# ViacheslavDanilov/oct_segmentation

Hardware: AMD Instinct MI355X
Metric: OCT frames/sec (704x704, bf16) fwd+bwd (higher is better)
Workload: dtype bf16; 1 GPU; unetplusplus/resnet101 1-class 704x704, batch 16/GPU, fwd+Dice+bwd+allreduce+Adam; global_batch=16, parallelism=dp1

## Files before the change

### oct_segmentation_amd/csrc/gemm1x1.hip

```cpp
#include "common.h"
#include "conv_common.h"
#include "kernels.h"

#include <cstdlib>
#include <type_traits>

namespace octseg {

constexpr int G1_BM = 128;
constexpr int G1_D = 3;
constexpr int G1_MAXWG = 512;

struct G1Args {
  const char* x; long long xstride;
  const float* scale; const float* shift; int relu;
  const char* w;
  char* y; long long ystride; int accum;
  int M, K, N, n_tiles, m_tiles;
  float* slab; int slab_row0;
  const float* bias; int relu_out;
};

template <typename T, int NT, bool AFF, bool BRES>
__global__ __launch_bounds__(256, BRES ? 1 : 2) void gemm1x1_kernel(const G1Args a) {
  constexpr int D = BRES ? 6 : G1_D;
  constexpr int NSET = D + 1;
  constexpr int NSLOT = BRES ? 4 : 2;
  constexpr int BN = NT * 32;
  constexpr int SLAB = BN * 128;
  constexpr int NPB = SLAB / 4096;
  constexpr int OPITCH = BN * 2 + 16;
  constexpr int PPR = BN / 8;
  constexpr int RPI = 64 / PPR;
  extern __shared__ __attribute__((aligned(16))) char smem[];
  char* ldsB = smem;
  char* strip0 = smem + NSLOT * SLAB;
  float* lds_ss = (float*)(strip0 + 4 * 32 * OPITCH);

  const int tid = threadIdx.x, lane = tid & 63, wave = tid >> 6;
  const int r = lane & 31, h = lane >> 5;
  const int G = gridDim.x;
  const int wid = blockIdx.x;
  const int l = (G & 7) == 0 ? (wid & 7) * (G >> 3) + (wid >> 3) : wid;
  const int nt_idx = l % a.n_tiles, wg_m = l / a.n_tiles, Gm = G / a.n_tiles;
  const int nloc = (a.m_tiles - wg_m + Gm - 1) / Gm;
  const int S = a.K >> 6;
  const int total = nloc * S;
  const int n0 = nt_idx * BN;

  if constexpr (AFF) {
    for (int k = tid; k < a.K; k += 256) { lds_ss[k] = a.scale[k]; lds_ss[a.K + k] = a.shift[k]; }
  }

  int pf_s = 0, pf_mt = wg_m;
  auto row_ptr = [&](int mt) -> const char* {
    const int row = min(mt * G1_BM + wave * 32 + r, a.M - 1);
    return a.x + (long long)row * a.xstride + 64 * h;
  };
  const char* pf_ptr = row_ptr(pf_mt);
  uint4 A[NSET][4];
  auto load_A = [&](uint4 (&dst)[4]) __attribute__((always_inline)) {
#pragma unroll
    for (int j = 0; j < 4; ++j) dst[j] = *(const uint4*)(pf_ptr + 16 * j);
    pf_ptr += 128;
    if (++pf_s == S) {
      pf_s = 0;
      if (pf_mt + Gm < a.m_tiles) pf_mt += Gm;
      pf_ptr = row_ptr(pf_mt);
    }
  };
  int bs = 0;
  const char* wbase = a.w + (long long)nt_idx * SLAB + tid * 16;
  const long long wstep = (long long)a.n_tiles * SLAB;
  uint4 B0 = make_uint4(0, 0, 0, 0), B1 = B0, B2 = B0, B3 = B0;
#define G1_LOAD_B()                                                        \
  do {                                                                     \
    const char* p_ = wbase + bs * wstep;                                   \
    B0 = *(const uint4*)(p_);                                              \
    if constexpr (NPB > 1) B1 = *(const uint4*)(p_ + 4096);                \
    if constexpr (NPB > 2) { B2 = *(const uint4*)(p_ + 8192); B3 = *(const uint4*)(p_ + 12288); } \
    if (++bs == S) bs = 0;                                                 \
  } while (0)
#define G1_STORE_B(slot_)                                                  \
  do {                                                                     \
    char* q_ = ldsB + (slot_) * SLAB + tid * 16;                           \
    *(uint4*)(q_) = B0;                                                    \
    if constexpr (NPB > 1) *(uint4*)(q_ + 4096) = B1;                      \
    if constexpr (NPB > 2) { *(uint4*)(q_ + 8192) = B2; *(uint4*)(q_ + 12288) = B3; } \
  } while (0)

  f32x16_t acc[NT];
#pragma unroll
  for (int nt = 0; nt < NT; ++nt)
#pragma unroll
    for (int v = 0; v < 16; ++v) acc[nt][v] = 0.f;
  float s1[NT], s2[NT];
#pragma unroll
  for (int nt = 0; nt < NT; ++nt) { s1[nt] = 0.f; s2[nt] = 0.f; }

  float obias[NT];
#pragma unroll
  for (int nt = 0; nt < NT; ++nt) obias[nt] = (a.bias != nullptr && n0 + nt * 32 + r < a.N) ? a.bias[n0 + nt * 32 + r] : 0.f;
  const float ofloor = a.relu_out ? 0.f : NO_FLOOR;
  const int bswz = (r >> 1) & 7;
  const int bbase = r * 128;
  const unsigned floor16 = a.relu ? 0u : 0x80008000u;

  if constexpr (BRES) {
    for (int q = 0; q < S; ++q) { G1_LOAD_B(); G1_STORE_B(q); }
  } else {
    G1_LOAD_B();
    G1_STORE_B(0);
    G1_LOAD_B();
  }
#pragma unroll
  for (int d = 0; d < D; ++d) load_A(A[d]);
  __syncthreads();

  int s = 0, mt = wg_m;
  char* strip = strip0 + wave * 32 * OPITCH;

  auto epilogue = [&]() __attribute__((always_inline)) {
    const int m0 = mt * G1_BM + wave * 32;
    if (a.bias != nullptr) {
#pragma unroll
      for (int nt = 0; nt < NT; ++nt)
#pragma unroll
        for (int v = 0; v < 16; ++v) acc[nt][v] = clamp_lo(acc[nt][v] + obias[nt], ofloor);
    }
    if (a.slab != nullptr) {
#pragma unroll
      for (int nt = 0; nt < NT; ++nt)
#pragma unroll
        for (int v = 0; v < 16; ++v) { const float y = acc[nt][v]; s1[nt] += y; s2[nt] += y * y; }
    }
#pragma unroll
    for (int nt = 0; nt < NT; ++nt)
#pragma unroll
      for (int v = 0; v < 16; ++v) {
        const int row = (v & 3) + 8 * (v >> 2) + 4 * h;
        Tr<T>::store(strip + row * OPITCH, nt * 32 + r, acc[nt][v]);
        acc[nt][v] = 0.f;
      }
    __builtin_amdgcn_fence(__ATOMIC_RELEASE, "wavefront");
    asm volatile("s_waitcnt lgkmcnt(0)" ::: "memory");
    const int piece = lane % PPR, rsub = lane / PPR;
    const int n = n0 + piece * 8;
    const bool nok = n < a.N;
    char* gp0 = a.y + (long long)(m0 + rsub) * a.ystride + n * 2;
    const long long gstep = (long long)RPI * a.ystride;
    if (a.accum) {
      uint4 old[32 / RPI];
#pragma unroll
      for (int i = 0; i < 32 / RPI; ++i) {
        const bool ok = nok && m0 + rsub + i * RPI < a.M;
        old[i] = *(const uint4*)(ok ? gp0 + i * gstep : (char*)a.y);
      }
#pragma unroll
      for (int i = 0; i < 32 / RPI; ++i) {
        const int row = rsub + i * RPI;
        if (nok && m0 + row < a.M) {
          const uint4 val = *(const uint4*)(strip + row * OPITCH + piece * 16);
          float x0[8], x1[8];
          Tr<T>::unpack8(val, x0); Tr<T>::unpack8(old[i], x1);
#pragma unroll
          for (int e = 0; e < 8; ++e) x0[e] += x1[e];
          *(uint4*)(gp0 + i * gstep) = Tr<T>::pack8(x0);
        }
      }
    } else {
#pragma unroll
      for (int i = 0; i < 32 / RPI; ++i) {
        const int row = rsub + i * RPI;
        if (nok && m0 + row < a.M) *(uint4*)(gp0 + i * gstep) = *(const uint4*)(strip + row * OPITCH + piece * 16);
      }
    }
    asm volatile("s_waitcnt lgkmcnt(0)" ::: "memory");
  };

  auto step = [&](auto set_c, int g) __attribute__((always_inline)) {
    constexpr int SET = decltype(set_c)::value;
    const int slot = BRES ? s : (g & 1);
    if constexpr (!BRES) {
      G1_STORE_B(slot ^ 1);
      G1_LOAD_B();
    }
    load_A(A[(SET + D) % NSET]);
    const bool tail = (mt * G1_BM + G1_BM > a.M);
    const bool valid = mt * G1_BM + wave * 32 + r < a.M;
    const char* bsl = ldsB + slot * SLAB + bbase;
    uint4 bf[2][NT];
#pragma unroll
    for (int nt = 0; nt < NT; ++nt) bf[0][nt] = *(const uint4*)(bsl + nt * 4096 + (((4 * h + 0) ^ bswz) * 16));
#pragma unroll
    for (int j = 0; j < 4; ++j) {
      if (j + 1 < 4) {
#pragma unroll
        for (int nt = 0; nt < NT; ++nt) bf[(j + 1) & 1][nt] = *(const uint4*)(bsl + nt * 4096 + (((4 * h + j + 1) ^ bswz) * 16));
      }
      uint4 af = A[SET][j];
      if constexpr (AFF) {
        const int k0 = s * 64 + 32 * h + 8 * j;
        float sc[8], sh[8];
        const float4 c0 = *(const float4*)(lds_ss + k0), c1 = *(const float4*)(lds_ss + k0 + 4);
        const float4 d0 = *(const float4*)(lds_ss + a.K + k0), d1 = *(const float4*)(lds_ss + a.K + k0 + 4);
        sc[0] = c0.x; sc[1] = c0.y; sc[2] = c0.z; sc[3] = c0.w; sc[4] = c1.x; sc[5] = c1.y; sc[6] = c1.z; sc[7] = c1.w;
        sh[0] = d0.x; sh[1] = d0.y; sh[2] = d0.z; sh[3] = d0.w; sh[4] = d1.x; sh[5] = d1.y; sh[6] = d1.z; sh[7] = d1.w;
        af = Tr<T>::affine_floor(af, sc, sh, floor16);
      }
      if (tail && !valid) af = make_uint4(0, 0, 0, 0);
      __builtin_amdgcn_sched_barrier(0);
#pragma unroll
      for (int nt = 0; nt < NT; ++nt) Tr<T>::mma(af, bf[j & 1][nt], acc[nt]);
      __builtin_amdgcn_sched_barrier(0);
    }
    if (++s == S) {
      epilogue();
      s = 0;
      mt += Gm;
    }
    if constexpr (!BRES) __syncthreads();
  };

  for (int g = 0; g < total; g += NSET) {
    step(std::integral_constant<int, 0>{}, g);
    if (g + 1 < total) step(std::integral_constant<int, 1>{}, g + 1);
    if (g + 2 < total) step(std::integral_constant<int, 2>{}, g + 2);
    if (g + 3 < total) step(std::integral_constant<int, 3>{}, g + 3);
    if constexpr (NSET > 4) {
      if (g + 4 < total) step(std::integral_constant<int, 4 % NSET>{}, g + 4);
      if (g + 5 < total) step(std::integral_constant<int, 5 % NSET>{}, g + 5);
      if (g + 6 < total) step(std::integral_constant<int, 6 % NSET>{}, g + 6);
    }
  }
  if constexpr (BRES) __syncthreads();

#undef G1_LOAD_B
#undef G1_STORE_B
  if (a.slab != nullptr) {
    float* red = (float*)strip0;
#pragma unroll
    for (int nt = 0; nt < NT; ++nt) {
      s1[nt] += __shfl_xor(s1[nt], 32);
      s2[nt] += __shfl_xor(s2[nt], 32);
      if (h == 0) { red[(wave * BN + nt * 32 + r) * 2] = s1[nt]; red[(wave * BN + nt * 32 + r) * 2 + 1] = s2[nt]; }
    }
    __syncthreads();
    if (tid < BN && n0 + tid < a.N) {
      float t1 = 0.f, t2 = 0.f;
#pragma unroll
      for (int w = 0; w < 4; ++w) { t1 += red[(w * BN + tid) * 2]; t2 += red[(w * BN + tid) * 2 + 1]; }
      float* o = a.slab + ((size_t)(a.slab_row0 + wg_m) * a.N + n0 + tid) * 2;
      o[0] = t1; o[1] = t2;
    }
  }
}

namespace {

struct G1Geom { int NT, n_tiles, m_tiles, G, rows, bres; size_t lds; };

static G1Geom g1_geom(const ConvArgs& a) {
  G1Geom g;
  g.NT = a.Cout > 64 ? 4 : (a.Cout > 32 ? 2 : 1);
  const int BN = g.NT * 32;
  g.n_tiles = (a.Cout + BN - 1) / BN;
  const long long M = (long long)a.N * a.OH * a.OW;
  g.m_tiles = (int)((M + G1_BM - 1) / G1_BM);
  static const bool use_bres = getenv("OCTSEG_G1_BRES") != nullptr;
  g.bres = (use_bres && g.NT == 4 && a.Cin <= 256 && a.Cin >= 128 && g.n_tiles >= 4) ? 1 : 0;
  int gm = (g.bres ? G1_MAXWG / 2 : G1_MAXWG) / g.n_tiles;
  if (gm < 1) gm = 1;
  if (gm > g.m_tiles) gm = g.m_tiles;
  g.rows = gm;
  g.G = gm * g.n_tiles;
  const bool aff = a.src[0].scale != nullptr;
  g.lds = (size_t)(g.bres ? 4 : 2) * BN * 128 + (size_t)4 * 32 * (BN * 2 + 16) + (aff ? (size_t)a.Cin * 8 : 0);
  return g;
}

}

bool gemm1x1_eligible(const ConvArgs& a, int dtype) {
  static const bool off = getenv("OCTSEG_NO_GEMM1X1") != nullptr;
  if (off || dtype == DT_F32) return false;
  if (a.ntaps != 1 || a.istride != 1 || a.ostride != 1 || a.out_mode == OUT_HEAD_NCHW) return false;
  if (a.tap_dy[0] != 0 || a.tap_dx[0] != 0 || a.nsrc != 1 || a.ndst != 1) return false;
  if (a.bias != nullptr && a.stat_slab != nullptr) return false;
  const SrcDesc& s = a.src[0];
  const DstDesc& d = a.dst[0];
  if (s.up || s.C != a.Cin || s.c0 != 0 || s.H != a.IH || s.W != a.IW || a.IH != a.OH || a.IW != a.OW) return false;
  if (d.pool || d.c0 != 0 || d.H != a.OH || d.W != a.OW || d.cn != a.Cout) return false;
  if (a.Cin % 64 != 0 || a.Cin > 4096 || a.Cout % 8 != 0 || a.Cout < 8) return false;
  if ((long long)a.N * a.OH * a.OW < 1) return false;
  return true;
}

int gemm1x1_rows(const ConvArgs& a) { return g1_geom(a).rows; }

template <typename T, int NT, bool AFF, bool BRES>
static hipError_t g1_launch_k(const G1Args& ga, const G1Geom& g, hipStream_t st) {
  static bool set = false;
  if (!set) {
    hipError_t e = hipFuncSetAttribute((const void*)gemm1x1_kernel<T, NT, AFF, BRES>, hipFuncAttributeMaxDynamicSharedMemorySize, 160 * 1024);
    if (e != hipSuccess) return e;
    set = true;
  }
  hipLaunchKernelGGL((gemm1x1_kernel<T, NT, AFF, BRES>), dim3(g.G), dim3(256), g.lds, st, ga);
  return hipGetLastError();
}
template <typename T, int NT>
static hipError_t g1_launch(const G1Args& ga, const G1Geom& g, bool aff, hipStream_t st) {
  if constexpr (NT == 4) {
    if (g.bres) return aff ? g1_launch_k<T, NT, true, true>(ga, g, st) : g1_launch_k<T, NT, false, true>(ga, g, st);
  }
  return aff ? g1_launch_k<T, NT, true, false>(ga, g, st) : g1_launch_k<T, NT, false, false>(ga, g, st);
}

hipError_t launch_gemm1x1(int dtype, const ConvArgs& a, hipStream_t st) {
  const G1Geom g = g1_geom(a);
  G1Args ga;
  const SrcDesc& s = a.src[0];
  const DstDesc& d = a.dst[0];
  ga.x = (const char*)s.ptr; ga.xstride = (long long)s.C * 2;
  ga.scale = s.scale; ga.shift = s.shift; ga.relu = s.relu;
  ga.w = (const char*)a.W;
  ga.y = (char*)d.ptr; ga.ystride = (long long)d.C * 2; ga.accum = (d.accum || a.out_mode == OUT_ACCUM) ? 1 : 0;
  ga.M = (int)((long long)a.N * a.OH * a.OW); ga.K = a.Cin; ga.N = a.Cout; ga.n_tiles = g.n_tiles; ga.m_tiles = g.m_tiles;
  ga.slab = a.stat_slab; ga.slab_row0 = a.slab_row0;
  ga.bias = a.bias; ga.relu_out = a.relu_out;
  const bool aff = s.scale != nullptr;
  if (dtype == DT_F16) {
    switch (g.NT) {
      case 4: return g1_launch<f16_t, 4>(ga, g, aff, st);
      case 2: return g1_launch<f16_t, 2>(ga, g, aff, st);
      default: return g1_launch<f16_t, 1>(ga, g, aff, st);
    }
  }
  switch (g.NT) {
    case 4: return g1_launch<bf16_t, 4>(ga, g, aff, st);
    case 2: return g1_launch<bf16_t, 2>(ga, g, aff, st);
    default: return g1_launch<bf16_t, 1>(ga, g, aff, st);
  }
}

}
```

Measured before the change: 254.9 frames/s.

## Add three-slot LDS ring with direct global-to-LDS weight loads in 1x1 GEMM

Adds a RING variant of the 1x1 GEMM kernel that streams weight tiles straight into a three-slot LDS ring using global_load_lds_dwordx4, skipping the register round trip. Activations are loaded with inline-asm global loads and waited on with explicit vmcnt counters, so each step needs only a single s_barrier. The epilogue strip is narrowed to write half the N tile at a time, which keeps LDS within the 80KB cap. It is enabled by default whenever it fits that cap. The hand-written waitcnt and m0 handling are fragile and depend on the exact order the compiler emits instructions.

```diff
diff --git a/oct_segmentation_amd/csrc/gemm1x1.hip b/oct_segmentation_amd/csrc/gemm1x1.hip
--- a/oct_segmentation_amd/csrc/gemm1x1.hip
+++ b/oct_segmentation_amd/csrc/gemm1x1.hip
@@ -21,23 +21,30 @@
   const float* bias; int relu_out;
 };
 
-template <typename T, int NT, bool AFF, bool BRES>
+constexpr int g1_ring_ew(int NT) { return NT == 4 ? 2 : NT; }
+constexpr int G1_RING_SLOTS = 3;
+constexpr size_t G1_RING_LDS_MAX = 80 * 1024;
+
+template <typename T, int NT, bool AFF, bool BRES, bool RING>
 __global__ __launch_bounds__(256, BRES ? 1 : 2) void gemm1x1_kernel(const G1Args a) {
+  static_assert(!(BRES && RING), "one weight pipeline per instantiation");
+  typedef __attribute__((ext_vector_type(4))) unsigned u32x4_t;
   constexpr int D = BRES ? 6 : G1_D;
   constexpr int NSET = D + 1;
-  constexpr int NSLOT = BRES ? 4 : 2;
+  constexpr int NSLOT = BRES ? 4 : (RING ? G1_RING_SLOTS : 2);
   constexpr int BN = NT * 32;
   constexpr int SLAB = BN * 128;
   constexpr int NPB = SLAB / 4096;
-  constexpr int OPITCH = BN * 2 + 16;
-  constexpr int PPR = BN / 8;
+  constexpr int EW = RING ? g1_ring_ew(NT) : NT;
+  constexpr int OPITCH = EW * 64 + 16;
+  constexpr int PPR = EW * 4;
   constexpr int RPI = 64 / PPR;
   extern __shared__ __attribute__((aligned(16))) char smem[];
   char* ldsB = smem;
   char* strip0 = smem + NSLOT * SLAB;
   float* lds_ss = (float*)(strip0 + 4 * 32 * OPITCH);
 
-  const int tid = threadIdx.x, lane = tid & 63, wave = tid >> 6;
+  const int tid = threadIdx.x, lane = tid & 63, wave = __builtin_amdgcn_readfirstlane(tid >> 6);
   const int r = lane & 31, h = lane >> 5;
   const int G = gridDim.x;
   const int wid = blockIdx.x;
@@ -69,9 +76,35 @@
       pf_ptr = row_ptr(pf_mt);
     }
   };
+  u32x4_t RA[NSET][4];
+  auto load_RA = [&](u32x4_t (&dst)[4]) __attribute__((always_inline)) {
+    asm volatile("global_load_dwordx4 %0, %1, off" : "=v"(dst[0]) : "v"(pf_ptr));
+    asm volatile("global_load_dwordx4 %0, %1, off offset:16" : "=v"(dst[1]) : "v"(pf_ptr));
+    asm volatile("global_load_dwordx4 %0, %1, off offset:32" : "=v"(dst[2]) : "v"(pf_ptr));
+    asm volatile("global_load_dwordx4 %0, %1, off offset:48" : "=v"(dst[3]) : "v"(pf_ptr));
+    pf_ptr += 128;
+    if (++pf_s == S) {
+      pf_s = 0;
+      if (pf_mt + Gm < a.m_tiles) pf_mt += Gm;
+      pf_ptr = row_ptr(pf_mt);
+    }
+  };
   int bs = 0;
   const char* wbase = a.w + (long long)nt_idx * SLAB + tid * 16;
   const long long wstep = (long long)a.n_tiles * SLAB;
+  const unsigned ldsB_addr = (unsigned)(size_t)(__attribute__((address_space(3))) char*)ldsB;
+  auto dma_B = [&](int slot) __attribute__((always_inline)) {
+    const char* p_ = wbase + bs * wstep;
+#pragma unroll
+    for (int i = 0; i < NPB; ++i) {
+      const char* g_ = p_ + i * 4096;
+      const unsigned dst = __builtin_amdgcn_readfirstlane(ldsB_addr + (unsigned)slot * SLAB + (unsigned)i * 4096u + (unsigned)wave * 1024u);
+      unsigned keep;
+      asm volatile("s_mov_b32 %0, m0\n\ts_mov_b32 m0, %2\n\ts_nop 0\n\tglobal_load_lds_dwordx4 %1, off\n\ts_mov_b32 m0, %0"
+                   : "=&s"(keep) : "v"(g_), "s"(dst) : "memory");
+    }
+    if (++bs == S) bs = 0;
+  };
   uint4 B0 = make_uint4(0, 0, 0, 0), B1 = B0, B2 = B0, B3 = B0;
 #define G1_LOAD_B()                                                        \
   do {                                                                     \
@@ -106,16 +139,29 @@
   const int bbase = r * 128;
   const unsigned floor16 = a.relu ? 0u : 0x80008000u;
 
-  if constexpr (BRES) {
-    for (int q = 0; q < S; ++q) { G1_LOAD_B(); G1_STORE_B(q); }
+  if constexpr (RING) {
+#pragma unroll
+    for (int nt = 0; nt < NT; ++nt) asm volatile("" : "+v"(obias[nt]));
+    asm volatile("s_waitcnt vmcnt(0)" ::: "memory");
+    load_RA(RA[0]); dma_B(0);
+    load_RA(RA[1]); dma_B(1);
+    load_RA(RA[2]);
+    asm volatile("s_waitcnt vmcnt(%4)" : "+v"(RA[0][0]), "+v"(RA[0][1]), "+v"(RA[0][2]), "+v"(RA[0][3]) : "n"(8 + NPB) : "memory");
+    asm volatile("s_waitcnt lgkmcnt(0)" ::: "memory");
+    __builtin_amdgcn_s_barrier();
+    asm volatile("" ::: "memory");
   } else {
-    G1_LOAD_B();
-    G1_STORE_B(0);
-    G1_LOAD_B();
-  }
-#pragma unroll
-  for (int d = 0; d < D; ++d) load_A(A[d]);
-  __syncthreads();
+    if constexpr (BRES) {
+      for (int q = 0; q < S; ++q) { G1_LOAD_B(); G1_STORE_B(q); }
+    } else {
+      G1_LOAD_B();
+      G1_STORE_B(0);
+      G1_LOAD_B();
+    }
+#pragma unroll
+    for (int d = 0; d < D; ++d) load_A(A[d]);
+    __syncthreads();
+  }
 
   int s = 0, mt = wg_m;
   char* strip = strip0 + wave * 32 * OPITCH;
@@ -135,17 +181,19 @@
         for (int v = 0; v < 16; ++v) { const float y = acc[nt][v]; s1[nt] += y; s2[nt] += y * y; }
     }
 #pragma unroll
-    for (int nt = 0; nt < NT; ++nt)
+    for (int ep = 0; ep < NT / EW; ++ep) {
+#pragma unroll
+    for (int e = 0; e < EW; ++e)
 #pragma unroll
       for (int v = 0; v < 16; ++v) {
         const int row = (v & 3) + 8 * (v >> 2) + 4 * h;
-        Tr<T>::store(strip + row * OPITCH, nt * 32 + r, acc[nt][v]);
-        acc[nt][v] = 0.f;
+        Tr<T>::store(strip + row * OPITCH, e * 32 + r, acc[ep * EW + e][v]);
+        acc[ep * EW + e][v] = 0.f;
       }
     __builtin_amdgcn_fence(__ATOMIC_RELEASE, "wavefront");
     asm volatile("s_waitcnt lgkmcnt(0)" ::: "memory");
     const int piece = lane % PPR, rsub = lane / PPR;
-    const int n = n0 + piece * 8;
+    const int n = n0 + ep * EW * 32 + piece * 8;
     const bool nok = n < a.N;
     char* gp0 = a.y + (long long)(m0 + rsub) * a.ystride + n * 2;
     const long long gstep = (long long)RPI * a.ystride;
@@ -168,6 +216,8 @@
           *(uint4*)(gp0 + i * gstep) = Tr<T>::pack8(x0);
         }
       }
+#pragma unroll
+      for (int i = 0; i < 32 / RPI; ++i) asm volatile("" :: "v"(old[i].x), "v"(old[i].y), "v"(old[i].z), "v"(old[i].w));
     } else {
 #pragma unroll
       for (int i = 0; i < 32 / RPI; ++i) {
@@ -176,16 +226,10 @@
       }
     }
     asm volatile("s_waitcnt lgkmcnt(0)" ::: "memory");
-  };
-
-  auto step = [&](auto set_c, int g) __attribute__((always_inline)) {
-    constexpr int SET = decltype(set_c)::value;
-    const int slot = BRES ? s : (g & 1);
-    if constexpr (!BRES) {
-      G1_STORE_B(slot ^ 1);
-      G1_LOAD_B();
-    }
-    load_A(A[(SET + D) % NSET]);
+    }
+  };
+
+  auto compute = [&](const uint4 (&a4)[4], int slot) __attribute__((always_inline)) {
     const bool tail = (mt * G1_BM + G1_BM > a.M);
     const bool valid = mt * G1_BM + wave * 32 + r < a.M;
     const char* bsl = ldsB + slot * SLAB + bbase;
@@ -198,7 +242,7 @@
 #pragma unroll
         for (int nt = 0; nt < NT; ++nt) bf[(j + 1) & 1][nt] = *(const uint4*)(bsl + nt * 4096 + (((4 * h + j + 1) ^ bswz) * 16));
       }
-      uint4 af = A[SET][j];
+      uint4 af = a4[j];
       if constexpr (AFF) {
         const int k0 = s * 64 + 32 * h + 8 * j;
         float sc[8], sh[8];
@@ -214,6 +258,17 @@
       for (int nt = 0; nt < NT; ++nt) Tr<T>::mma(af, bf[j & 1][nt], acc[nt]);
       __builtin_amdgcn_sched_barrier(0);
     }
+  };
+
+  auto step = [&](auto set_c, int g) __attribute__((always_inline)) {
+    constexpr int SET = decltype(set_c)::value;
+    const int slot = BRES ? s : (g & 1);
+    if constexpr (!BRES) {
+      G1_STORE_B(slot ^ 1);
+      G1_LOAD_B();
+    }
+    load_A(A[(SET + D) % NSET]);
+    compute(A[SET], slot);
     if (++s == S) {
       epilogue();
       s = 0;
@@ -222,6 +277,42 @@
     if constexpr (!BRES) __syncthreads();
   };
 
+  int rslot = 0, wslot = 2;
+  auto rstep = [&](auto set_c, bool live) __attribute__((always_inline)) {
+    constexpr int SET = decltype(set_c)::value;
+    constexpr int NXT = (SET + 1) % NSET;
+    dma_B(wslot);
+    if (++wslot == NSLOT) wslot = 0;
+    load_RA(RA[(SET + D) % NSET]);
+    uint4 a4[4];
+#pragma unroll
+    for (int j = 0; j < 4; ++j) a4[j] = __builtin_bit_cast(uint4, RA[SET][j]);
+    if (live) compute(a4, rslot);
+    if (++rslot == NSLOT) rslot = 0;
+    asm volatile("s_waitcnt vmcnt(%4)" : "+v"(RA[NXT][0]), "+v"(RA[NXT][1]), "+v"(RA[NXT][2]), "+v"(RA[NXT][3]) : "n"(8 + NPB) : "memory");
+    if (live && ++s == S) {
+      epilogue();
+      s = 0;
+      mt += Gm;
+    }
+    asm volatile("s_waitcnt lgkmcnt(0)" ::: "memory");
+    __builtin_amdgcn_s_barrier();
+    asm volatile("" ::: "memory");
+  };
+
+  if constexpr (RING) {
+    static_assert(NSET == 4, "the unrolled ring walk below");
+    for (int g = 0; g < total; g += NSET) {
+      rstep(std::integral_constant<int, 0>{}, true);
+      rstep(std::integral_constant<int, 1>{}, g + 1 < total);
+      rstep(std::integral_constant<int, 2>{}, g + 2 < total);
+      rstep(std::integral_constant<int, 3>{}, g + 3 < total);
+    }
+    asm volatile("s_waitcnt vmcnt(0)"
+                 : "+v"(RA[0][0]), "+v"(RA[0][1]), "+v"(RA[0][2]), "+v"(RA[0][3]), "+v"(RA[1][0]), "+v"(RA[1][1]), "+v"(RA[1][2]), "+v"(RA[1][3]),
+                   "+v"(RA[2][0]), "+v"(RA[2][1]), "+v"(RA[2][2]), "+v"(RA[2][3]), "+v"(RA[3][0]), "+v"(RA[3][1]), "+v"(RA[3][2]), "+v"(RA[3][3])
+                 :: "memory");
+  } else
   for (int g = 0; g < total; g += NSET) {
     step(std::integral_constant<int, 0>{}, g);
     if (g + 1 < total) step(std::integral_constant<int, 1>{}, g + 1);
@@ -258,7 +349,11 @@
 
 namespace {
 
-struct G1Geom { int NT, n_tiles, m_tiles, G, rows, bres; size_t lds; };
+struct G1Geom { int NT, n_tiles, m_tiles, G, rows, bres, ring; size_t lds; };
+
+static size_t g1_lds_bytes(int NT, int slots, int ew, bool aff, int K) {
+  return (size_t)slots * NT * 32 * 128 + (size_t)4 * 32 * (ew * 64 + 16) + (aff ? (size_t)K * 8 : 0);
+}
 
 static G1Geom g1_geom(const ConvArgs& a) {
   G1Geom g;
@@ -275,7 +370,10 @@
   g.rows = gm;
   g.G = gm * g.n_tiles;
   const bool aff = a.src[0].scale != nullptr;
-  g.lds = (size_t)(g.bres ? 4 : 2) * BN * 128 + (size_t)4 * 32 * (BN * 2 + 16) + (aff ? (size_t)a.Cin * 8 : 0);
+  static const bool no_ring = getenv("OCTSEG_G1_NO_RING") != nullptr;
+  const size_t ring_lds = g1_lds_bytes(g.NT, G1_RING_SLOTS, g1_ring_ew(g.NT), aff, a.Cin);
+  g.ring = (!no_ring && !g.bres && ring_lds <= G1_RING_LDS_MAX) ? 1 : 0;
+  g.lds = g.ring ? ring_lds : g1_lds_bytes(g.NT, g.bres ? 4 : 2, g.NT, aff, a.Cin);
   return g;
 }
 
@@ -298,23 +396,24 @@
 
 int gemm1x1_rows(const ConvArgs& a) { return g1_geom(a).rows; }
 
-template <typename T, int NT, bool AFF, bool BRES>
+template <typename T, int NT, bool AFF, bool BRES, bool RING>
 static hipError_t g1_launch_k(const G1Args& ga, const G1Geom& g, hipStream_t st) {
   static bool set = false;
   if (!set) {
-    hipError_t e = hipFuncSetAttribute((const void*)gemm1x1_kernel<T, NT, AFF, BRES>, hipFuncAttributeMaxDynamicSharedMemorySize, 160 * 1024);
+    hipError_t e = hipFuncSetAttribute((const void*)gemm1x1_kernel<T, NT, AFF, BRES, RING>, hipFuncAttributeMaxDynamicSharedMemorySize, 160 * 1024);
     if (e != hipSuccess) return e;
     set = true;
   }
-  hipLaunchKernelGGL((gemm1x1_kernel<T, NT, AFF, BRES>), dim3(g.G), dim3(256), g.lds, st, ga);
+  hipLaunchKernelGGL((gemm1x1_kernel<T, NT, AFF, BRES, RING>), dim3(g.G), dim3(256), g.lds, st, ga);
   return hipGetLastError();
 }
 template <typename T, int NT>
 static hipError_t g1_launch(const G1Args& ga, const G1Geom& g, bool aff, hipStream_t st) {
   if constexpr (NT == 4) {
-    if (g.bres) return aff ? g1_launch_k<T, NT, true, true>(ga, g, st) : g1_launch_k<T, NT, false, true>(ga, g, st);
-  }
-  return aff ? g1_launch_k<T, NT, true, false>(ga, g, st) : g1_launch_k<T, NT, false, false>(ga, g, st);
+    if (g.bres) return aff ? g1_launch_k<T, NT, true, true, false>(ga, g, st) : g1_launch_k<T, NT, false, true, false>(ga, g, st);
+  }
+  if (g.ring) return aff ? g1_launch_k<T, NT, true, false, true>(ga, g, st) : g1_launch_k<T, NT, false, false, true>(ga, g, st);
+  return aff ? g1_launch_k<T, NT, true, false, false>(ga, g, st) : g1_launch_k<T, NT, false, false, false>(ga, g, st);
 }
 
 hipError_t launch_gemm1x1(int dtype, const ConvArgs& a, hipStream_t st) {
```

Result: no change. 254.5 frames/s (-0.2%).
